# aquaskyline/Clairvoyante

Hardware: AMD Instinct MI355X
Metric: candidate tensors/sec (higher is better)
Workload: dtype f32

## Files before the change

### clairvoyante_amd/csrc/cv_kernels_conv.hpp

```cpp
#pragma once

template <int P, bool ACT = false>
__device__ __forceinline__ unsigned pool_code4(const f4 (&older)[P > 1 ? P - 1 : 1], f4 v, f4 o)
{
    unsigned c = 0;
#pragma unroll
    for (int r = 0; r < 4; r++) {
        int idx = P - 1;
#pragma unroll
        for (int d = P - 2; d >= 0; d--) {
            bool hit = older[d][r] == o[r];
            if constexpr (ACT) hit = hit && __builtin_signbit(older[d][r]) == __builtin_signbit(o[r]);
            idx = hit ? d : idx;
        }
        (void)v;
        c |= (unsigned)idx << (4 * r);
    }
    return c;
}

template <int POOL, bool SAVE = false>
__global__ __launch_bounds__(256) void conv1_tm(const float *__restrict__ x, int64_t n,
                                                 const float *__restrict__ wp1,
                                                 const float *__restrict__ bias, int cout,
                                                 f4 *__restrict__ out_tm, int G, u32x2 *__restrict__ code_tm = nullptr)
{
    constexpr int HIN = CV_INPUT_H, HOUT = HIN - POOL + 1, SPLIT = 4;
    const int lane = threadIdx.x & 63;
    const int wv = blockIdx.x * 4 + (threadIdx.x >> 6);
    const int g = wv / SPLIT, part = wv % SPLIT;
    if (g >= G) return;
    const int r0 = (HOUT * part) / SPLIT, r1 = (HOUT * (part + 1)) / SPLIT;
    const int c = lane & 15, q = lane >> 4;
    int64_t cand = (int64_t)g * 16 + c;
    if (cand >= n) cand = n - 1;
    const float *xp = x + (size_t)cand * (HIN * 16) + q;
    float A[4];
#pragma unroll
    for (int kw = 0; kw < 4; kw++) A[kw] = wp1[kw * 64 + lane];
    const f4 b4 = load_bias4(bias, 0, q, cout);
    f4 pw[POOL > 1 ? POOL - 1 : 1][4];
#pragma unroll
    for (int j = 0; j < (POOL > 1 ? POOL - 1 : 1); j++)
#pragma unroll
        for (int w = 0; w < 4; w++) pw[j][w] = (f4){0.f, 0.f, 0.f, 0.f};
    float xw[4], xn[4];
#pragma unroll
    for (int w = 0; w < 4; w++) xw[w] = xp[r0 * 16 + w * 4];
    f4 *op = out_tm + (size_t)g * HOUT * 4 * 64 + lane;
    const int hend = r1 + POOL - 1;
#pragma unroll 1
    for (int h = r0; h < hend; h++) {
        {
            const int hn = h + 1 < hend ? h + 1 : h;
#pragma unroll
            for (int w = 0; w < 4; w++) xn[w] = xp[hn * 16 + w * 4];
        }
        f4 acc[4];
#pragma unroll
        for (int w = 0; w < 4; w++) acc[w] = (f4){0.f, 0.f, 0.f, 0.f};
#pragma unroll
        for (int kw = 0; kw < 4; kw++)
#pragma unroll
            for (int wo = 0; wo < 4; wo++) {
                const int wi = wo + kw - 1;
                if (wi < 0 || wi > 3) continue;
                acc[wo] = mfma4(A[kw], xw[wi], acc[wo]);
            }
        if constexpr (!SAVE && POOL > 1) {
#pragma unroll
            for (int w = 0; w < 4; w++) {
                const f4 t = acc[w] + b4;
                const f4 o = max4(pw[POOL - 2][w], t);
#pragma unroll
                for (int j = POOL - 2; j > 0; j--) pw[j][w] = max4(pw[j - 1][w], t);
                pw[0][w] = t;
                if (h - r0 >= POOL - 1) op[(size_t)((h - (POOL - 1)) * 4 + w) * 64] = selu4(o);
            }
#pragma unroll
            for (int w = 0; w < 4; w++) xw[w] = xn[w];
            continue;
        }
        f4 v[4];
#pragma unroll
        for (int w = 0; w < 4; w++) v[w] = selu4(acc[w] + b4);
        if constexpr (POOL > 1) {
            f4 o[4];
#pragma unroll
            for (int w = 0; w < 4; w++) {
                o[w] = v[w];
#pragma unroll
                for (int j = 0; j < POOL - 1; j++) o[w] = max4(o[w], pw[j][w]);
            }
            if constexpr (SAVE) {
                if (h - r0 >= POOL - 1) {
                    unsigned cw[4];
#pragma unroll
                    for (int w = 0; w < 4; w++) {
                        f4 older[POOL - 1];
#pragma unroll
                        for (int j = 0; j < POOL - 1; j++) older[j] = pw[j][w];
                        cw[w] = pool_code4<POOL, true>(older, v[w], o[w]);
                    }
                    code_tm[((size_t)g * HOUT + (h - (POOL - 1))) * 64 + lane] = (u32x2){cw[0] | (cw[1] << 16), cw[2] | (cw[3] << 16)};
                }
            }
#pragma unroll
            for (int j = 0; j + 1 < POOL - 1; j++)
#pragma unroll
                for (int w = 0; w < 4; w++) pw[j][w] = pw[j + 1][w];
#pragma unroll
            for (int w = 0; w < 4; w++) pw[POOL - 2][w] = v[w];
            if (h - r0 >= POOL - 1) {
#pragma unroll
                for (int w = 0; w < 4; w++) op[(size_t)((h - (POOL - 1)) * 4 + w) * 64] = o[w];
            }
        } else {
#pragma unroll
            for (int w = 0; w < 4; w++) op[(size_t)(h * 4 + w) * 64] = v[w];
        }
#pragma unroll
        for (int w = 0; w < 4; w++) xw[w] = xn[w];
    }
}

__device__ __forceinline__ f4 selu4_low(f4 v)
{
    const cvm::f2v a = cvm::selu2((cvm::f2v){v[0], v[1]});
    return (f4){a[0], a[1], 0.0f, 0.0f};
}

template <int FRONT, bool HALF = false>
struct front_source {
    static constexpr int NP = FRONT > 1 ? FRONT - 1 : 1;
    const float *xp;
    float A[4];
    f4 b4;
    f4 cw[NP][4];
    float xc[4], xn[4];
    int hx;

    __device__ __forceinline__ void load_x(float (&dst)[4], int h)
    {
        if (h < CV_INPUT_H) {
#pragma unroll
            for (int w = 0; w < 4; w++) dst[w] = xp[h * 16 + w * 4];
        }
    }
    __device__ __forceinline__ void conv1_row(f4 (&v)[4])
    {
        f4 acc[4];
#pragma unroll
        for (int w = 0; w < 4; w++) acc[w] = (f4){0.f, 0.f, 0.f, 0.f};
#pragma unroll
        for (int kw = 0; kw < 4; kw++)
#pragma unroll
            for (int wo = 0; wo < 4; wo++) {
                const int wi = wo + kw - 1;
                if (wi < 0 || wi > 3) continue;
                acc[wo] = mfma4(A[kw], xc[wi], acc[wo]);
            }
#pragma unroll
        for (int w = 0; w < 4; w++) v[w] = acc[w] + b4;
#pragma unroll
        for (int w = 0; w < 4; w++) xc[w] = xn[w];
        hx++;
        load_x(xn, hx + 1);
    }
    __device__ __forceinline__ void init(const float *x, int64_t cand, int q, const float *wp1,
                                         const float *bias1, int cout1, int lane, int h0 = 0)
    {
        xp = x + (size_t)cand * (CV_INPUT_H * 16) + q;
#pragma unroll
        for (int kw = 0; kw < 4; kw++) A[kw] = wp1[kw * 64 + lane];
        b4 = load_bias4(bias1, 0, q, cout1);
        hx = h0;
        load_x(xc, h0);
        load_x(xn, h0 + 1);
        if constexpr (FRONT > 1) {
#pragma unroll
            for (int r = 0; r < FRONT - 1; r++) {
                f4 v[4];
                conv1_row(v);
#pragma unroll
                for (int w = 0; w < 4; w++) {
#pragma unroll
                    for (int j = FRONT - 2; j > 0; j--) cw[j][w] = r == 0 ? v[w] : max4(cw[j - 1][w], v[w]);
                    cw[0][w] = v[w];
                }
            }
        }
    }
    __device__ __forceinline__ void next(f4 (&row)[4][1])
    {
        f4 v[4];
        conv1_row(v);
        if constexpr (FRONT > 1) {
#pragma unroll
            for (int w = 0; w < 4; w++) {
                const f4 o = max4(cw[FRONT - 2][w], v[w]);
#pragma unroll
                for (int j = FRONT - 2; j > 0; j--) cw[j][w] = max4(cw[j - 1][w], v[w]);
                cw[0][w] = v[w];
                row[w][0] = HALF ? selu4_low(o) : selu4(o);
            }
        } else {
#pragma unroll
            for (int w = 0; w < 4; w++) row[w][0] = HALF ? selu4_low(v[w]) : selu4(v[w]);
        }
    }
};

#define CV_CONV_XCD_UNITS(W) ((W) != 1 && (W) != 2 && (W) != 4)
template <int KH, int CINB, int NT, int POOL, int HIN, int FRONT, int MODE, int HSPLIT = 1, int KS4 = 4>
__global__ __launch_bounds__(256, 2) void conv_tm(const f4 *__restrict__ in_tm, const float *__restrict__ x,
                                                   int64_t n, const float *__restrict__ wp1,
                                                   const float *__restrict__ bias1, int cout1,
                                                   const f4 *__restrict__ wp, const float *__restrict__ bias,
                                                   int cout, f4 *__restrict__ out_tm, f4 *__restrict__ act_tm, int G,
                                                   int rows_per = 0)
{
    static_assert(FRONT == 0 || CINB == 1, "the fused first layer feeds one 16-channel fragment");
    static_assert(MODE != 2 || (POOL == 1 && FRONT == 0), "the data-gradient pass has no pooling / first layer");
    static_assert(HSPLIT >= 1 || FRONT == 0, "flat ranges read their rows from a TM buffer (position parts may make them: front_source::init h0)");
    static_assert(HSPLIT != 0 || (FRONT == 0 && (MODE != 0 || POOL == 1)), "flat ranges: training kernels, and inference layers without pooling (slim small passes)");
    extern __shared__ __attribute__((aligned(16))) f4 ldsw[];
    constexpr int PADT = MODE == 2 ? KH - 1 - (KH - 1) / 2 : (KH - 1) / 2;
    constexpr int PADL = MODE == 2 ? 2 : 1;
    constexpr int HOUT = HIN - POOL + 1;
    constexpr int NFRAG = NT * KH * 4 * CINB;
    for (int i = threadIdx.x; i < NFRAG * 64; i += 256) ldsw[i] = wp[i];
    __syncthreads();
    const int lane = threadIdx.x & 63;
    int wv = __builtin_amdgcn_readfirstlane(blockIdx.x * 4 + (threadIdx.x >> 6));
    if constexpr (HSPLIT >= 1 && CV_CONV_XCD_UNITS(NT * HSPLIT)) {
        if (gridDim.x >= 16) {
            const int x = blockIdx.x & 7;
            const int lw = __builtin_amdgcn_readfirstlane((blockIdx.x >> 3) * 4 + (threadIdx.x >> 6));
            wv = ((lw / (NT * HSPLIT)) * 8 + x) * (NT * HSPLIT) + lw % (NT * HSPLIT);
        }
    }
    constexpr int HSD = HSPLIT > 0 ? HSPLIT : 1;
    int nt, gF, gL, hs = 0, r0 = 0, r1 = 0;
    if constexpr (HSPLIT == 0) {
        nt = wv % NT;
        r0 = (wv / NT) * rows_per;
        r1 = r0 + rows_per < G * HOUT ? r0 + rows_per : G * HOUT;
        if (r0 >= r1) return;
        gF = r0 / HOUT; gL = (r1 - 1) / HOUT;
    } else {
        const int gt = wv / HSD;
        hs = wv % HSD; nt = gt % NT; gF = gL = gt / NT;
        if (gF >= G) return;
    }
    CV_STAMP_BEGIN
    const int q = lane >> 4;
    const f4 b4 = MODE == 2 ? (f4){0.f, 0.f, 0.f, 0.f} : load_bias4(bias, nt, q, cout);
    const f4 *wl = ldsw + (size_t)nt * (KH * 4 * CINB * 64) + lane;
#pragma unroll 1
    for (int g = gF; g <= gL; g++) {
    int hbeg, hend;
    if constexpr (HSPLIT == 0) {
        const int oa = r0 - g * HOUT > 0 ? r0 - g * HOUT : 0, ob = r1 - g * HOUT < HOUT ? r1 - g * HOUT : HOUT;
        hbeg = oa; hend = POOL > 1 ? ob + POOL - 1 : ob;
    } else {
        hbeg = POOL > 1 ? HOUT * hs / HSD : HIN * hs / HSD;
        hend = POOL > 1 ? HOUT * (hs + 1) / HSD + POOL - 1 : HIN * (hs + 1) / HSD;
    }
    const f4 *inp = in_tm + (size_t)g * (HIN * 4 * CINB * 64) + lane;
    f4 *op = out_tm + (size_t)g * (HOUT * 4 * NT * 64) + (size_t)nt * 64 + lane;

    front_source<FRONT, (KS4 <= 2)> fs;
    if constexpr (FRONT > 0) {
        int64_t cand = (int64_t)g * 16 + (lane & 15);
        if (cand >= n) cand = n - 1;
        fs.init(x, cand, q, wp1, bias1, cout1, lane, hbeg - PADT > 0 ? hbeg - PADT : 0);
    }
    auto fetch_row = [&](int hr, f4 (&row)[4][CINB]) {
        if constexpr (FRONT > 0) {
            fs.next(row);
        } else {
#pragma unroll
            for (int w = 0; w < 4; w++)
#pragma unroll
                for (int cb = 0; cb < CINB; cb++) row[w][cb] = inp[(size_t)((hr * 4 + w) * CINB + cb) * 64];
        }
    };
    constexpr bool SPREAD = FRONT == 0;
    static_assert(CINB <= 3, "the counted wait below names at most 12 fragments");
    const f4 *const inp_s = in_tm + (size_t)__builtin_amdgcn_readfirstlane(g) * (HIN * 4 * CINB * 64);
    const unsigned lane16 = (unsigned)lane * 16u;
    auto load_piece = [&](int hr, int w, int cb, f4 &dst) {
        const f4 *ps = inp_s + (size_t)((hr * 4 + w) * CINB + cb) * 64;
        asm volatile("global_load_dwordx4 %0, %1, %2" : "=v"(dst) : "v"(lane16), "s"(ps));
    };

    f4 win[KH][4][CINB];
    f4 nxt[4][CINB];
    f4 pw[POOL > 1 ? POOL - 1 : 1][4];
    const f4 zero = (f4){0.f, 0.f, 0.f, 0.f};
#pragma unroll
    for (int j = 0; j < (POOL > 1 ? POOL - 1 : 1); j++)
#pragma unroll
        for (int w = 0; w < 4; w++) pw[j][w] = zero;
#pragma unroll
    for (int j = 0; j < KH; j++) {
        const int hr = hbeg + j - PADT;
        f4 tmp[4][CINB];
#pragma unroll
        for (int w = 0; w < 4; w++)
#pragma unroll
            for (int cb = 0; cb < CINB; cb++) tmp[w][cb] = zero;
        if (hr >= 0 && hr < HIN) fetch_row(hr, tmp);
#pragma unroll
        for (int w = 0; w < 4; w++)
#pragma unroll
            for (int cb = 0; cb < CINB; cb++) {
                if (j < KH - 1) win[j][w][cb] = tmp[w][cb]; else nxt[w][cb] = tmp[w][cb];
            }
    }
#pragma unroll 1
    for (int h = hbeg; h < hend; h++) {
#pragma unroll
        for (int w = 0; w < 4; w++)
#pragma unroll
            for (int cb = 0; cb < CINB; cb++) win[KH - 1][w][cb] = nxt[w][cb];
        {
            const int hr = h + 1 + (KH - 1) - PADT;
            if (!SPREAD && hr < HIN) fetch_row(hr, nxt);
        }
        const int hnext = h + 1 + (KH - 1) - PADT < HIN ? h + 1 + (KH - 1) - PADT : HIN - 1;
        f4 acc[4];
#pragma unroll
        for (int w = 0; w < 4; w++) acc[w] = zero;
#pragma unroll
        for (int kh = 0; kh < KH; kh++) {
            const int hr = h + kh - PADT;
            const bool on = hr >= 0 && hr < HIN;
            if (on) {
#pragma unroll
                for (int kw = 0; kw < 4; kw++)
#pragma unroll
                    for (int cb = 0; cb < CINB; cb++) {
                        const f4 A = wl[(size_t)((kh * 4 + kw) * CINB + cb) * 64];
#pragma unroll
                        for (int s = 0; s < KS4; s++)
#pragma unroll
                            for (int wo = 0; wo < 4; wo++) {
                                const int wi = wo + kw - PADL;
                                if (wi < 0 || wi > 3) continue;
                                acc[wo] = mfma4(A[s], win[kh][wi][cb][s], acc[wo]);
                            }
                        if constexpr (SPREAD) {
                            if (kh == 0) load_piece(hnext, kw, cb, nxt[kw][cb]);
                        }
                    }
            } else if (SPREAD && kh == 0) {
#pragma unroll
                for (int kw = 0; kw < 4; kw++)
#pragma unroll
                    for (int cb = 0; cb < CINB; cb++) load_piece(hnext, kw, cb, nxt[kw][cb]);
            }
        }
        if constexpr (SPREAD) {
            {
                if constexpr (CINB == 1)
                    asm volatile("s_waitcnt vmcnt(0)" : "+v"(nxt[0][0]), "+v"(nxt[1][0]), "+v"(nxt[2][0]), "+v"(nxt[3][0]) : : "memory");
                else if constexpr (CINB == 2)
                    asm volatile("s_waitcnt vmcnt(0)" : "+v"(nxt[0][0]), "+v"(nxt[1][0]), "+v"(nxt[2][0]), "+v"(nxt[3][0]),
                                 "+v"(nxt[0][1]), "+v"(nxt[1][1]), "+v"(nxt[2][1]), "+v"(nxt[3][1]) : : "memory");
                else
                    asm volatile("s_waitcnt vmcnt(0)" : "+v"(nxt[0][0]), "+v"(nxt[1][0]), "+v"(nxt[2][0]), "+v"(nxt[3][0]),
                                 "+v"(nxt[0][1]), "+v"(nxt[1][1]), "+v"(nxt[2][1]), "+v"(nxt[3][1]),
                                 "+v"(nxt[0][CINB - 1]), "+v"(nxt[1][CINB - 1]), "+v"(nxt[2][CINB - 1]), "+v"(nxt[3][CINB - 1]) : : "memory");
            }
        }
        if constexpr (MODE == 0 && POOL > 1) {
#pragma unroll
            for (int w = 0; w < 4; w++) {
                const f4 t = acc[w] + b4;
                const f4 o = max4(pw[POOL - 2][w], t);
#pragma unroll
                for (int j = POOL - 2; j > 0; j--) pw[j][w] = max4(pw[j - 1][w], t);
                pw[0][w] = t;
                if (h - hbeg >= POOL - 1) {
                    op[(size_t)((h - (POOL - 1)) * 4 + w) * (NT * 64)] = selu4(o);
                }
            }
#pragma unroll
            for (int j = 0; j + 1 < KH; j++)
#pragma unroll
                for (int w = 0; w < 4; w++)
#pragma unroll
                    for (int cb = 0; cb < CINB; cb++) win[j][w][cb] = win[j + 1][w][cb];
            continue;
        }
        f4 v[4];
        if constexpr (MODE == 2) {
#pragma unroll
            for (int w = 0; w < 4; w++) v[w] = acc[w];
            if (act_tm) {
                const f4 *yp = act_tm + (size_t)g * (HOUT * 4 * NT * 64) + (size_t)nt * 64 + lane;
#pragma unroll
                for (int w = 0; w < 4; w++) {
                    const f4 y = yp[(size_t)(h * 4 + w) * (NT * 64)];
#pragma unroll
                    for (int k = 0; k < 4; k++) v[w][k] *= cv_selu_grad_from_out(y[k]);
                }
            }
        } else {
#pragma unroll
            for (int w = 0; w < 4; w++) v[w] = selu4(acc[w] + b4);
        }
        if constexpr (POOL > 1) {
            f4 o[4];
#pragma unroll
            for (int w = 0; w < 4; w++) {
                o[w] = v[w];
#pragma unroll
                for (int j = 0; j < POOL - 1; j++) o[w] = max4(o[w], pw[j][w]);
            }
            if constexpr (MODE == 1) {
                if (h - hbeg >= POOL - 1) {
                    unsigned cw[4];
#pragma unroll
                    for (int w = 0; w < 4; w++) {
                        f4 older[POOL - 1];
#pragma unroll
                        for (int j = 0; j < POOL - 1; j++) older[j] = pw[j][w];
                        cw[w] = pool_code4<POOL, true>(older, v[w], o[w]);
                    }
                    u32x2 *cp = reinterpret_cast<u32x2 *>(act_tm);
                    cp[(((size_t)g * HOUT + (h - (POOL - 1))) * NT + nt) * 64 + lane] = (u32x2){cw[0] | (cw[1] << 16), cw[2] | (cw[3] << 16)};
                }
            }
#pragma unroll
            for (int j = 0; j + 1 < POOL - 1; j++)
#pragma unroll
                for (int w = 0; w < 4; w++) pw[j][w] = pw[j + 1][w];
#pragma unroll
            for (int w = 0; w < 4; w++) pw[POOL - 2][w] = v[w];
            if (h - hbeg >= POOL - 1) {
#pragma unroll
                for (int w = 0; w < 4; w++) op[(size_t)((h - (POOL - 1)) * 4 + w) * (NT * 64)] = o[w];
            }
        } else {
#pragma unroll
            for (int w = 0; w < 4; w++) op[(size_t)(h * 4 + w) * (NT * 64)] = v[w];
        }
#pragma unroll
        for (int j = 0; j + 1 < KH; j++)
#pragma unroll
            for (int w = 0; w < 4; w++)
#pragma unroll
                for (int cb = 0; cb < CINB; cb++) win[j][w][cb] = win[j + 1][w][cb];
    }
    }
    CV_STAMP_END(MODE == 2 && KH == 3 && CINB == 3, 2);
    CV_STAMP_END(MODE == 1 && KH == 2 && CINB == 1 && FRONT == 0, 6);
}

template <int CH, bool FLAT = false>
__global__ __launch_bounds__(FLAT ? 128 : 256, 2) void front2_tm(const float *__restrict__ x, int64_t n,
                                                     const float *__restrict__ wp1, const float *__restrict__ bias1,
                                                     int cout1, const f4 *__restrict__ wp,
                                                     const float *__restrict__ bias, int cout,
                                                     f4 *__restrict__ out_tm, int G, int rows_per = 0)
{
    constexpr int P1 = 5, H1 = CV_INPUT_H - P1 + 1;
    constexpr int NT = 2, P2 = 4, H2 = H1 - P2 + 1;
    constexpr int NW = NT * 2 * 4 * 64;
    extern __shared__ __attribute__((aligned(16))) f4 lds[];
    f4 *rows = lds + NW;
    for (int i = threadIdx.x; i < NW; i += (FLAT ? 128 : 256)) lds[i] = wp[i];
    const int lane = threadIdx.x & 63, wid = threadIdx.x >> 6;
    const int gl = FLAT ? 0 : wid >> 1, nt = wid & 1;
    int gF, gL, r0 = 0, r1 = 0;
    bool live = true;
    if constexpr (FLAT) {
        r0 = (int)blockIdx.x * rows_per;
        r1 = r0 + rows_per < G * H2 ? r0 + rows_per : G * H2;
        if (r0 >= r1) return;
        gF = r0 / H2; gL = (r1 - 1) / H2;
    } else {
        const int gq = blockIdx.x * 2 + gl;
        live = gq < G;
        gF = gL = live ? gq : G - 1;
    }
    const int q = lane >> 4;
    float A1[4];
#pragma unroll
    for (int kw = 0; kw < 4; kw++) A1[kw] = wp1[kw * 64 + lane];
    const f4 b1 = load_bias4(bias1, 0, q, cout1);
    const f4 b2 = load_bias4(bias, nt, q, cout);
    const f4 *wl = lds + (size_t)nt * (2 * 4 * 64) + lane;
    f4 *myrows = rows + (size_t)gl * (CH * 4 * 64) + lane;
    const f4 zero = (f4){0.f, 0.f, 0.f, 0.f};
    f4 prev[4], m1[4], m2[4], m3[4];
#pragma unroll
    for (int w = 0; w < 4; w++) { prev[w] = zero; m1[w] = zero; m2[w] = zero; m3[w] = zero; }
    __syncthreads();
    CV_PHASE_BEGIN
#pragma unroll 1
    for (int g = gF; g <= gL; g++) {
    int oa = 0, ob = H2;
    if constexpr (FLAT) {
        oa = r0 - g * H2 > 0 ? r0 - g * H2 : 0;
        ob = r1 - g * H2 < H2 ? r1 - g * H2 : H2;
    }
    const int pend = ob + P2 < H1 ? ob + P2 : H1;
    int64_t cand = (int64_t)g * 16 + (lane & 15);
    if (cand >= n) cand = n - 1;
    const float *xp = x + (size_t)cand * (CV_INPUT_H * 16) + q;
    f4 *op = out_tm + (size_t)g * (H2 * 4 * NT * 64) + (size_t)nt * 64 + lane;

    auto out_row = [&](int h, const f4 (&cur)[4], bool has_cur) {
        f4 acc[4];
#pragma unroll
        for (int w = 0; w < 4; w++) acc[w] = zero;
#pragma unroll
        for (int kw = 0; kw < 4; kw++) {
            const f4 A = wl[(size_t)(0 * 4 + kw) * 64];
#pragma unroll
            for (int s4 = 0; s4 < 4; s4++)
#pragma unroll
                for (int wo = 0; wo < 4; wo++) {
                    const int wi = wo + kw - 1;
                    if (wi < 0 || wi > 3) continue;
                    acc[wo] = mfma4(A[s4], prev[wi][s4], acc[wo]);
                }
        }
        if (has_cur) {
#pragma unroll
            for (int kw = 0; kw < 4; kw++) {
                const f4 A = wl[(size_t)(1 * 4 + kw) * 64];
#pragma unroll
                for (int s4 = 0; s4 < 4; s4++)
#pragma unroll
                    for (int wo = 0; wo < 4; wo++) {
                        const int wi = wo + kw - 1;
                        if (wi < 0 || wi > 3) continue;
                        acc[wo] = mfma4(A[s4], cur[wi][s4], acc[wo]);
                    }
            }
        }
#pragma unroll
        for (int w = 0; w < 4; w++) {
            const f4 t = acc[w] + b2;
            const f4 o = max4(m3[w], t);
            m3[w] = max4(m2[w], t);
            m2[w] = max4(m1[w], t);
            m1[w] = t;
            if (h - oa >= P2 - 1 && live) op[(size_t)((h - (P2 - 1)) * 4 + w) * (NT * 64)] = selu4(o);
        }
    };

#pragma unroll 1
    for (int c0 = oa; c0 < pend; c0 += CH) {
        const int cn = pend - c0 < CH ? pend - c0 : CH;
        const int half = (cn + 1) >> 1;
        const int a0 = c0 + nt * half;
        const int a1 = a0 + half < c0 + cn ? a0 + half : c0 + cn;
        if (a0 < a1) {
            static_assert(CH == 6, "the block pooling below is written for three rows per wave");
            constexpr int HALF = CH / 2, NRAW = HALF + P1 - 1;
            float xr[NRAW][4];
#pragma unroll
            for (int r = 0; r < NRAW; r++) {
                const int rr = a0 + r < CV_INPUT_H ? a0 + r : CV_INPUT_H - 1;
#pragma unroll
                for (int w = 0; w < 4; w++) xr[r][w] = xp[rr * 16 + w * 4];
            }
            CV_PHASE(0);
            CV_PHASE_DRAIN();
            CV_PHASE(3);
            f4 t[NRAW][4];
#pragma unroll
            for (int r = 0; r < NRAW; r++) {
                f4 acc[4];
#pragma unroll
                for (int w = 0; w < 4; w++) acc[w] = zero;
#pragma unroll
                for (int kw = 0; kw < 4; kw++)
#pragma unroll
                    for (int wo = 0; wo < 4; wo++) {
                        const int wi = wo + kw - 1;
                        if (wi < 0 || wi > 3) continue;
                        acc[wo] = mfma4(A1[kw], xr[r][wi], acc[wo]);
                    }
#pragma unroll
                for (int w = 0; w < 4; w++) t[r][w] = acc[w] + b1;
            }
#pragma unroll
            for (int w = 0; w < 4; w++) {
                const f4 c = max3_4(t[2][w], t[3][w], t[4][w]);
                const f4 o0 = max3_4(t[0][w], t[1][w], c);
                const f4 o1 = max3_4(t[1][w], c, t[5][w]);
                const f4 o2 = max3_4(c, t[5][w], t[6][w]);
                myrows[(size_t)((a0 - c0 + 0) * 4 + w) * 64] = selu4(o0);
                if (a0 + 1 < a1) myrows[(size_t)((a0 - c0 + 1) * 4 + w) * 64] = selu4(o1);
                if (a0 + 2 < a1) myrows[(size_t)((a0 - c0 + 2) * 4 + w) * 64] = selu4(o2);
            }
        }
        CV_PHASE(0);
        __syncthreads();
        CV_PHASE(2);
#pragma unroll 1
        for (int p = c0; p < c0 + cn; p++) {
            f4 cur[4];
#pragma unroll
            for (int w = 0; w < 4; w++) cur[w] = myrows[(size_t)((p - c0) * 4 + w) * 64];
            if (p > oa) out_row(p - 1, cur, true);
#pragma unroll
            for (int w = 0; w < 4; w++) prev[w] = cur[w];
        }
        CV_PHASE(1);
        __syncthreads();
        CV_PHASE(2);
    }
    if (ob == H2) out_row(H1 - 1, prev, false);
    }
    CV_PHASE(1);
    CV_PHASE_END(true, wid);
}

template <int CINB, int NT, int HIN, int WAVES, int MINW, bool SAVE = false>
__global__ __launch_bounds__(WAVES * 64, MINW) void conv3_rot(const f4 *__restrict__ in_tm, const f4 *__restrict__ wp,
                                                            const float *__restrict__ bias, int cout,
                                                            f4 *__restrict__ out_tm, int G, u32x2 *__restrict__ code_tm = nullptr,
                                                            int rows_per = 0)
{
    constexpr int KH = 3, PADT = 1, POOL = 3, HOUT = HIN - POOL + 1;
    extern __shared__ __attribute__((aligned(16))) f4 ldsw[];
    constexpr int NFRAG = NT * KH * 4 * CINB;
    for (int i = threadIdx.x; i < NFRAG * 64; i += WAVES * 64) ldsw[i] = wp[i];
    __syncthreads();
    const int lane = threadIdx.x & 63;
    int wv = __builtin_amdgcn_readfirstlane(blockIdx.x * WAVES + (threadIdx.x >> 6));
    const bool flat = rows_per > 0;
    if (gridDim.x >= 16) {
        const int x = blockIdx.x & 7;
        const int lw = __builtin_amdgcn_readfirstlane((blockIdx.x >> 3) * WAVES + (threadIdx.x >> 6));
        wv = ((lw / NT) * 8 + x) * NT + lw % NT;
    }
    const int nt = wv % NT;
    int gF = wv / NT, gL = gF, r0 = 0, r1 = 0;
    if (flat) {
        r0 = (wv / NT) * rows_per;
        r1 = r0 + rows_per < G * HOUT ? r0 + rows_per : G * HOUT;
        if (r0 >= r1) return;
        gF = r0 / HOUT; gL = (r1 - 1) / HOUT;
    } else if (gF >= G) return;
    CV_STAMP_BEGIN
    const int q = lane >> 4;
    const f4 b4 = load_bias4(bias, nt, q, cout);
    const f4 *wl = ldsw + (size_t)nt * (KH * 4 * CINB * 64) + lane;
    const f4 zero = (f4){0.f, 0.f, 0.f, 0.f};
    const unsigned lane16 = (unsigned)lane * 16u;
#pragma unroll 1
    for (int g = gF; g <= gL; g++) {
    int hbeg = 0, hend = HIN;
    if (flat) {
        hbeg = r0 - g * HOUT > 0 ? r0 - g * HOUT : 0;
        hend = (r1 - g * HOUT < HOUT ? r1 - g * HOUT : HOUT) + POOL - 1;
    }
    const f4 *inp = in_tm + (size_t)g * (HIN * 4 * CINB * 64) + lane;
    f4 *op = out_tm + (size_t)g * (HOUT * 4 * NT * 64) + (size_t)nt * 64 + lane;
    f4 win[3][4][CINB];
    f4 tp[3][4];
#pragma unroll
    for (int j = 0; j < 3; j++)
#pragma unroll
        for (int w = 0; w < 4; w++) tp[j][w] = zero;
    auto load_row = [&](int hr, f4 (&row)[4][CINB]) {
#pragma unroll
        for (int w = 0; w < 4; w++)
#pragma unroll
            for (int cb = 0; cb < CINB; cb++) row[w][cb] = inp[(size_t)((hr * 4 + w) * CINB + cb) * 64];
    };
    load_row(hbeg, win[1]);
    if (hbeg > 0) load_row(hbeg - 1, win[0]);
    static_assert(CINB == 2, "the counted wait below names 8 fragments");
    const f4 *const inp_s = in_tm + (size_t)g * (HIN * 4 * CINB * 64);
    auto load_piece = [&](int hr, int w, int cb, f4 &dst) {
        const f4 *ps = inp_s + (size_t)((hr * 4 + w) * CINB + cb) * 64;
        asm volatile("global_load_dwordx4 %0, %1, %2" : "=v"(dst) : "v"(lane16), "s"(ps));
    };
    auto step = [&](auto Rc, int h) {
        constexpr int R = decltype(Rc)::value;
        const int hnext = h + 1 < HIN ? h + 1 : HIN - 1;
        f4 acc[4];
#pragma unroll
        for (int w = 0; w < 4; w++) acc[w] = zero;
#pragma unroll
        for (int kh = 0; kh < KH; kh++) {
            const int hr = h + kh - PADT;
            const bool on = hr >= 0 && hr < HIN;
            if (kh == KH - 1) {
                f4 (&nw)[4][CINB] = win[(R + 2) % 3];
                asm volatile("s_waitcnt vmcnt(0)" : "+v"(nw[0][0]), "+v"(nw[1][0]), "+v"(nw[2][0]), "+v"(nw[3][0]),
                             "+v"(nw[0][1]), "+v"(nw[1][1]), "+v"(nw[2][1]), "+v"(nw[3][1]) : : "memory");
            }
            if (on) {
#pragma unroll
                for (int kw = 0; kw < 4; kw++)
#pragma unroll
                    for (int cb = 0; cb < CINB; cb++) {
                        const f4 A = wl[(size_t)((kh * 4 + kw) * CINB + cb) * 64];
#pragma unroll
                        for (int s = 0; s < 4; s++)
#pragma unroll
                            for (int wo = 0; wo < 4; wo++) {
                                const int wi = wo + kw - 1;
                                if (wi < 0 || wi > 3) continue;
                                acc[wo] = mfma4(A[s], win[(R + kh) % 3][wi][cb][s], acc[wo]);
                            }
                        if (kh == 0) load_piece(hnext, kw, cb, win[(R + 2) % 3][kw][cb]);
                    }
            } else if (kh == 0) {
#pragma unroll
                for (int kw = 0; kw < 4; kw++)
#pragma unroll
                    for (int cb = 0; cb < CINB; cb++) load_piece(hnext, kw, cb, win[(R + 2) % 3][kw][cb]);
            }
        }
#pragma unroll
        for (int w = 0; w < 4; w++) {
            if constexpr (SAVE) tp[R][w] = selu4(acc[w] + b4);
            else tp[R][w] = acc[w] + b4;
            if (h - hbeg >= POOL - 1) {
                if constexpr (SAVE) op[(size_t)((h - (POOL - 1)) * 4 + w) * (NT * 64)] = max3_4(tp[0][w], tp[1][w], tp[2][w]);
                else op[(size_t)((h - (POOL - 1)) * 4 + w) * (NT * 64)] = selu4(max3_4(tp[0][w], tp[1][w], tp[2][w]));
            }
        }
        if constexpr (SAVE) {
            if (h - hbeg >= POOL - 1) {
                unsigned cw[4];
#pragma unroll
                for (int w = 0; w < 4; w++) {
                    const f4 older[2] = {tp[(R + 1) % 3][w], tp[(R + 2) % 3][w]};
                    cw[w] = pool_code4<3, true>(older, tp[R][w], max3_4(tp[0][w], tp[1][w], tp[2][w]));
                }
                code_tm[(((size_t)g * HOUT + (h - (POOL - 1))) * NT + nt) * 64 + lane] = (u32x2){cw[0] | (cw[1] << 16), cw[2] | (cw[3] << 16)};
            }
        }
    };
#pragma unroll 1
    for (int h0 = hbeg; h0 < hend; h0 += 3) {
        step(std::integral_constant<int, 0>{}, h0);
        __builtin_amdgcn_sched_barrier(0);
        if (h0 + 1 < hend) step(std::integral_constant<int, 1>{}, h0 + 1);
        __builtin_amdgcn_sched_barrier(0);
        if (h0 + 2 < hend) step(std::integral_constant<int, 2>{}, h0 + 2);
        __builtin_amdgcn_sched_barrier(0);
    }
    }
    CV_STAMP_END(SAVE, 1);
}
```

Baseline: 18.57 million.

## Split front2 conv1 work by output column and carry pooling halo across chunks

Each wave pair now divides the first conv+pool stage by output columns (two per wave) rather than by rows. Each wave carries the last four conv1 rows in registers across chunks, so the pooling halo is no longer recomputed. The raw input for the next chunk is prefetched before the barrier so the load overlaps the second stage. This removes the redundant halo MFMAs and the load latency on the critical path, at the cost of more live registers and code duplicated per template column variant.

Measured after the change: 18.79 million, median of 6. 1.01x the previous value.

```diff
diff --git a/clairvoyante_amd/csrc/cv_kernels_conv.hpp b/clairvoyante_amd/csrc/cv_kernels_conv.hpp
--- a/clairvoyante_amd/csrc/cv_kernels_conv.hpp
+++ b/clairvoyante_amd/csrc/cv_kernels_conv.hpp
@@ -460,6 +460,8 @@
     CV_STAMP_END(MODE == 1 && KH == 2 && CINB == 1 && FRONT == 0, 6);
 }
 
+__device__ constexpr int f2col(int nt, int j) { return nt == 0 ? 1 + j : 3 * j; }
+
 template <int CH, bool FLAT = false>
 __global__ __launch_bounds__(FLAT ? 128 : 256, 2) void front2_tm(const float *__restrict__ x, int64_t n,
                                                      const float *__restrict__ wp1, const float *__restrict__ bias1,
@@ -555,53 +557,83 @@
         }
     };
 
+    static_assert(CH == 6, "the block pooling below is written for six rows per chunk");
+    f4 tc[P1 - 1][2];
+    float xn[CH][4];
+    const bool first = __builtin_amdgcn_readfirstlane(nt) == 0;
+    auto load_raw = [&](int row0) {
+#pragma unroll
+        for (int r = 0; r < CH; r++) {
+            const int rr = row0 + r < CV_INPUT_H ? row0 + r : CV_INPUT_H - 1;
+#pragma unroll
+            for (int w = 0; w < 4; w++) xn[r][w] = xp[rr * 16 + w * 4];
+        }
+    };
+    auto conv1_row = [&](auto NTc, const float (&xr)[4], f4 (&t)[2]) {
+#pragma unroll
+        for (int j = 0; j < 2; j++) {
+            constexpr int N = decltype(NTc)::value;
+            const int wo = f2col(N, j);
+            f4 acc = zero;
+#pragma unroll
+            for (int kw = 0; kw < 4; kw++) {
+                const int wi = wo + kw - 1;
+                if (wi < 0 || wi > 3) continue;
+                acc = mfma4(A1[kw], xr[wi], acc);
+            }
+            t[j] = acc + b1;
+        }
+    };
+    auto phase_a = [&](auto NTc, int cn) {
+        constexpr int N = decltype(NTc)::value;
+        f4 t[CH + P1 - 1][2];
+#pragma unroll
+        for (int r = 0; r < P1 - 1; r++)
+#pragma unroll
+            for (int j = 0; j < 2; j++) t[r][j] = tc[r][j];
+#pragma unroll
+        for (int r = 0; r < CH; r++) conv1_row(NTc, xn[r], t[P1 - 1 + r]);
+#pragma unroll
+        for (int j = 0; j < 2; j++) {
+            const int w = f2col(N, j);
+            const f4 c1 = max3_4(t[2][j], t[3][j], t[4][j]);
+            const f4 c2 = max3_4(t[5][j], t[6][j], t[7][j]);
+            const f4 o[CH] = {max3_4(t[0][j], t[1][j], c1), max3_4(t[1][j], c1, t[5][j]), max3_4(c1, t[5][j], t[6][j]),
+                              max3_4(t[3][j], t[4][j], c2), max3_4(t[4][j], c2, t[8][j]), max3_4(c2, t[8][j], t[9][j])};
+#pragma unroll
+            for (int i = 0; i < CH; i++)
+                if (i < cn) myrows[(size_t)(i * 4 + w) * 64] = selu4(o[i]);
+        }
+#pragma unroll
+        for (int r = 0; r < P1 - 1; r++)
+#pragma unroll
+            for (int j = 0; j < 2; j++) tc[r][j] = t[CH + r][j];
+    };
+    {
+        float xw[P1 - 1][4];
+#pragma unroll
+        for (int r = 0; r < P1 - 1; r++)
+#pragma unroll
+            for (int w = 0; w < 4; w++) xw[r][w] = xp[(oa + r) * 16 + w * 4];
+        load_raw(oa + P1 - 1);
+        if (first) {
+#pragma unroll
+            for (int r = 0; r < P1 - 1; r++) conv1_row(std::integral_constant<int, 0>{}, xw[r], tc[r]);
+        } else {
+#pragma unroll
+            for (int r = 0; r < P1 - 1; r++) conv1_row(std::integral_constant<int, 1>{}, xw[r], tc[r]);
+        }
+    }
+
 #pragma unroll 1
     for (int c0 = oa; c0 < pend; c0 += CH) {
         const int cn = pend - c0 < CH ? pend - c0 : CH;
-        const int half = (cn + 1) >> 1;
-        const int a0 = c0 + nt * half;
-        const int a1 = a0 + half < c0 + cn ? a0 + half : c0 + cn;
-        if (a0 < a1) {
-            static_assert(CH == 6, "the block pooling below is written for three rows per wave");
-            constexpr int HALF = CH / 2, NRAW = HALF + P1 - 1;
-            float xr[NRAW][4];
-#pragma unroll
-            for (int r = 0; r < NRAW; r++) {
-                const int rr = a0 + r < CV_INPUT_H ? a0 + r : CV_INPUT_H - 1;
-#pragma unroll
-                for (int w = 0; w < 4; w++) xr[r][w] = xp[rr * 16 + w * 4];
-            }
-            CV_PHASE(0);
-            CV_PHASE_DRAIN();
-            CV_PHASE(3);
-            f4 t[NRAW][4];
-#pragma unroll
-            for (int r = 0; r < NRAW; r++) {
-                f4 acc[4];
-#pragma unroll
-                for (int w = 0; w < 4; w++) acc[w] = zero;
-#pragma unroll
-                for (int kw = 0; kw < 4; kw++)
-#pragma unroll
-                    for (int wo = 0; wo < 4; wo++) {
-                        const int wi = wo + kw - 1;
-                        if (wi < 0 || wi > 3) continue;
-                        acc[wo] = mfma4(A1[kw], xr[r][wi], acc[wo]);
-                    }
-#pragma unroll
-                for (int w = 0; w < 4; w++) t[r][w] = acc[w] + b1;
-            }
-#pragma unroll
-            for (int w = 0; w < 4; w++) {
-                const f4 c = max3_4(t[2][w], t[3][w], t[4][w]);
-                const f4 o0 = max3_4(t[0][w], t[1][w], c);
-                const f4 o1 = max3_4(t[1][w], c, t[5][w]);
-                const f4 o2 = max3_4(c, t[5][w], t[6][w]);
-                myrows[(size_t)((a0 - c0 + 0) * 4 + w) * 64] = selu4(o0);
-                if (a0 + 1 < a1) myrows[(size_t)((a0 - c0 + 1) * 4 + w) * 64] = selu4(o1);
-                if (a0 + 2 < a1) myrows[(size_t)((a0 - c0 + 2) * 4 + w) * 64] = selu4(o2);
-            }
-        }
+        CV_PHASE(0);
+        CV_PHASE_DRAIN();
+        CV_PHASE(3);
+        if (first) phase_a(std::integral_constant<int, 0>{}, cn);
+        else phase_a(std::integral_constant<int, 1>{}, cn);
+        if (c0 + CH < pend) load_raw(c0 + CH + P1 - 1);
         CV_PHASE(0);
         __syncthreads();
         CV_PHASE(2);
```
